# ubc-vision/COTR

Hardware: AMD Instinct MI355X
Metric: query-correspondences/sec at 256x512 SBS, 1k queries (higher is better)
Workload: dtype f32

## Files before the change

cotr_amd/csrc/attention.hip:

```cpp
#include "common.h"

#define ATT_KEYS 512
#define ATT_HD 32

struct AttnFuse {
  const float* x;
  const float* x2;
  const float* wq;
  const float* bq;
  float qscale;
  const float* wo;
  float* part;
  int rows_total;
  int wt;
  unsigned long long* dbg;
};

template <int NS, int QP, bool OP>
__global__ __launch_bounds__(NS * 64) void attention_kernel(const float* __restrict__ q, int ldq,
                                                            const float* __restrict__ k,
                                                            const float* __restrict__ v, int ldkv,
                                                            float* __restrict__ o, int ldo, int nq, int head_major,
                                                            const AttnFuse fz) {
  static_assert(!(QP || OP) || NS == 4 || NS == 8, "the fused variants are written for 4 or 8 key splits");
  constexpr int NBO = 8 / (NS >= 4 ? NS : 4);
  constexpr int SLD = 32 * (NBO > 0 ? NBO : 1) + 4;
  constexpr int QCH = 256 / (NS >= 4 ? NS : 4);
  constexpr int NBLK = ATT_KEYS / NS / 32;
  constexpr int RPW = 16 / NS;
  constexpr int LDS_BUF = OP ? (NS * 32 * SLD > NS * 16 * 64 ? NS * 32 * SLD : NS * 16 * 64) : NS * 16 * 64;
  __shared__ __attribute__((aligned(16))) float lds_buf[LDS_BUF];
  float (*lds_o)[16][64] = reinterpret_cast<float (*)[16][64]>(lds_buf);
  __shared__ float lds_m[NS][32];
  __shared__ float lds_l[NS][32];
  __shared__ __attribute__((aligned(16))) float lds_out[32][36];

  const int t = threadIdx.x;
  const int lane = t & 63, wave = t >> 6;
  const int l31 = lane & 31, hh = lane >> 5;
#define ATT_STAMP(slot)                                                                                                        \
  do {                                                                                                                         \
    if (fz.dbg != nullptr && t == 0) fz.dbg[((size_t)blockIdx.z * gridDim.x + blockIdx.x) * 8 + (slot)] = wall_clock64();      \
  } while (0)
  ATT_STAMP(0);
  const int qtiles = gridDim.x >> 3;
  const int head = head_major ? (blockIdx.x & 7) : (blockIdx.x / qtiles);
  const int qtile = head_major ? (blockIdx.x >> 3) : (blockIdx.x % qtiles);
  const int pair = blockIdx.z;
  const int qi = qtile * 32 + l31;
  const bool q_ok = qi < nq;
  const size_t qrow = (size_t)pair * nq + (q_ok ? qi : 0);

  const size_t key0 = (size_t)pair * ATT_KEYS + (size_t)wave * (ATT_KEYS / NS);
  const float* kg = k + (key0 + l31) * ldkv + head * ATT_HD + hh * 4;
  const float* vg = v + (key0 + 4 * hh) * ldkv + head * ATT_HD + l31;
  f32x4 kf[4];
#pragma unroll
  for (int j = 0; j < 4; ++j) kf[j] = *reinterpret_cast<const f32x4*>(kg + j * 8);
  f32x4 wof[NBO > 0 ? NBO : 1][4];
  if constexpr (OP) {
#pragma unroll
    for (int nb = 0; nb < NBO; ++nb) {
      const float* worow = fz.wo + (size_t)((wave * NBO + nb) * 32 + l31) * 256 + head * ATT_HD + hh * 4;
#pragma unroll
      for (int j = 0; j < 4; ++j) wof[nb][j] = *reinterpret_cast<const f32x4*>(worow + j * 8);
    }
  }

  f32x4 qf[4];
  if constexpr (QP) {
    f32x4 bq4[4];
#pragma unroll
    for (int j = 0; j < 4; ++j) bq4[j] = *reinterpret_cast<const f32x4*>(fz.bq + head * ATT_HD + j * 8 + hh * 4);
    f32x16 qacc;
#pragma unroll
    for (int r = 0; r < 16; ++r) qacc[r] = 0.f;
    constexpr int QJ = QCH / 8;
    const float* wrow = fz.wq + (size_t)(head * ATT_HD + l31) * 256 + wave * QCH + hh * 4;
    const float* xrow = fz.x + qrow * 256 + wave * QCH + hh * 4;
    f32x4 wa[QJ], xb[QJ];
#pragma unroll
    for (int j = 0; j < QJ; ++j) wa[j] = *reinterpret_cast<const f32x4*>(wrow + j * 8);
#pragma unroll
    for (int j = 0; j < QJ; ++j) xb[j] = *reinterpret_cast<const f32x4*>(xrow + j * 8);
    if constexpr (QP == 2) {
      const float* x2row = fz.x2 + qrow * 256 + wave * QCH + hh * 4;
      f32x4 x2b[QJ];
#pragma unroll
      for (int j = 0; j < QJ; ++j) x2b[j] = *reinterpret_cast<const f32x4*>(x2row + j * 8);
#pragma unroll
      for (int j = 0; j < QJ; ++j) xb[j] += x2b[j];
    }
#pragma unroll
    for (int j = 0; j < QJ; ++j)
#pragma unroll
      for (int e = 0; e < 4; ++e) qacc = __builtin_amdgcn_mfma_f32_32x32x2f32(wa[j][e], xb[j][e], qacc, 0, 0, 0);
#pragma unroll
    for (int r = 0; r < 16; ++r) lds_o[wave][r][lane] = qacc[r];
    __syncthreads();
#pragma unroll
    for (int j = 0; j < 4; ++j)
#pragma unroll
      for (int e = 0; e < 4; ++e) {
        const int r = j * 4 + e;
        float sum = 0.f;
#pragma unroll
        for (int w = 0; w < NS; ++w) sum += lds_o[w][r][lane];
        sum += bq4[j][e];
        qf[j][e] = sum * fz.qscale * 1.44269504088896340736f;
      }
    __syncthreads();
    ATT_STAMP(1);
  } else {
#pragma unroll
    for (int j = 0; j < 4; ++j) {
      const f32x4 z = {0.f, 0.f, 0.f, 0.f};
      qf[j] = q_ok ? *reinterpret_cast<const f32x4*>(q + qrow * ldq + head * ATT_HD + j * 8 + hh * 4) : z;
      qf[j] *= 1.44269504088896340736f;
    }
  }
  f32x16 oacc;
#pragma unroll
  for (int r = 0; r < 16; ++r) oacc[r] = 0.f;
  float m_run = -INFINITY, l_run = 0.f;

#pragma unroll
  for (int kb = 0; kb < NBLK; ++kb) {
    float vf[16];
#pragma unroll
    for (int r = 0; r < 16; ++r) vf[r] = vg[(size_t)(kb * 32 + (r & 3) + 8 * (r >> 2)) * ldkv];
    f32x16 s;
#pragma unroll
    for (int r = 0; r < 16; ++r) s[r] = 0.f;
    __builtin_amdgcn_s_setprio(1);
#pragma unroll
    for (int j = 0; j < 4; ++j)
#pragma unroll
      for (int e = 0; e < 4; ++e) s = __builtin_amdgcn_mfma_f32_32x32x2f32(kf[j][e], qf[j][e], s, 0, 0, 0);
    if (kb + 1 < NBLK) {
#pragma unroll
      for (int j = 0; j < 4; ++j) kf[j] = *reinterpret_cast<const f32x4*>(kg + (size_t)(kb + 1) * 32 * ldkv + j * 8);
    }
    __builtin_amdgcn_s_setprio(0);
    float mx = s[0];
#pragma unroll
    for (int r = 1; r < 16; ++r) mx = fmaxf(mx, s[r]);
    mx = fmaxf(mx, __shfl_xor(mx, 32));
    const float m_new = fmaxf(m_run, mx);
    const float alpha = __builtin_amdgcn_exp2f(m_run - m_new);
    float psum = 0.f;
#pragma unroll
    for (int r = 0; r < 16; ++r) {
      s[r] = __builtin_amdgcn_exp2f(s[r] - m_new);
      psum += s[r];
    }
    l_run = l_run * alpha + psum;
    m_run = m_new;
#pragma unroll
    for (int r = 0; r < 16; ++r) oacc[r] *= alpha;
    __builtin_amdgcn_s_setprio(1);
#pragma unroll
    for (int r = 0; r < 16; ++r) oacc = __builtin_amdgcn_mfma_f32_32x32x2f32(vf[r], s[r], oacc, 0, 0, 0);
    __builtin_amdgcn_s_setprio(0);
  }
  l_run += __shfl_xor(l_run, 32);
  ATT_STAMP(2);

#pragma unroll
  for (int r = 0; r < 16; ++r) lds_o[wave][r][lane] = oacc[r];
  if (hh == 0) {
    lds_m[wave][l31] = m_run;
    lds_l[wave][l31] = l_run;
  }
  __syncthreads();
  float m_all = lds_m[0][l31];
#pragma unroll
  for (int w = 1; w < NS; ++w) m_all = fmaxf(m_all, lds_m[w][l31]);
  float f[NS];
  float l_all = 0.f;
#pragma unroll
  for (int w = 0; w < NS; ++w) {
    f[w] = __builtin_amdgcn_exp2f(lds_m[w][l31] - m_all);
    l_all += f[w] * lds_l[w][l31];
  }
  const float inv = 1.f / l_all;
#pragma unroll
  for (int i = 0; i < RPW; ++i) {
    const int r = wave * RPW + i;
    float acc = 0.f;
#pragma unroll
    for (int w = 0; w < NS; ++w) acc += f[w] * lds_o[w][r][lane];
    lds_out[l31][(r & 3) + 8 * (r >> 2) + 4 * hh] = acc * inv;
  }
  __syncthreads();
  ATT_STAMP(3);
  if constexpr (OP) {
    float* stage = lds_buf + wave * (32 * SLD);
    f32x4 af[4];
#pragma unroll
    for (int j = 0; j < 4; ++j) af[j] = *reinterpret_cast<const f32x4*>(&lds_out[l31][j * 8 + hh * 4]);
#pragma unroll
    for (int nb = 0; nb < NBO; ++nb) {
      f32x16 pacc;
#pragma unroll
      for (int r = 0; r < 16; ++r) pacc[r] = 0.f;
#pragma unroll
      for (int j = 0; j < 4; ++j)
#pragma unroll
        for (int e = 0; e < 4; ++e) pacc = __builtin_amdgcn_mfma_f32_32x32x2f32(af[j][e], wof[nb][j][e], pacc, 0, 0, 0);
#pragma unroll
      for (int r = 0; r < 16; ++r) stage[((r & 3) + 8 * (r >> 2) + 4 * hh) * SLD + nb * 32 + l31] = pacc[r];
    }
    ATT_STAMP(4);
    float* pbase = fz.part + ((size_t)head * fz.rows_total + (size_t)pair * nq) * 256 + wave * (32 * NBO);
    constexpr int LPR = 8 * NBO;
    constexpr int RPI = 64 / LPR;
    const int sr = lane / LPR, sc = (lane % LPR) * 4;
#pragma unroll
    for (int it = 0; it < 32 / RPI; ++it) {
      const int row = it * RPI + sr;
      const int qo = qtile * 32 + row;
      const f32x4 val = *reinterpret_cast<const f32x4*>(&stage[row * SLD + sc]);
      if (qo < nq) store_f32x4(pbase + (size_t)qo * 256 + sc, val, fz.wt != 0);
    }
    ATT_STAMP(5);
    if (o == nullptr) return;
  }
  for (int i = t; i < 256; i += NS * 64) {
    const int row = i >> 3, c4 = (i & 7) * 4;
    const int qo = qtile * 32 + row;
    if (qo < nq)
      *reinterpret_cast<f32x4*>(o + ((size_t)pair * nq + qo) * ldo + head * ATT_HD + c4) =
          *reinterpret_cast<const f32x4*>(&lds_out[row][c4]);
  }
}


template <int NS, int OCC>
__global__ __launch_bounds__(NS * 64, OCC) void attention_wide_kernel(const float* __restrict__ q, int ldq,
                                                                 const float* __restrict__ k,
                                                                 const float* __restrict__ v, int ldkv,
                                                                 float* __restrict__ o, int ldo, int nq, int head_major) {
  constexpr int NBLK = ATT_KEYS / NS / 32;
  constexpr int RPW = 16 / NS;
  __shared__ __attribute__((aligned(16))) float lds_o[NS][2][16][64];
  __shared__ float lds_m[NS][2][32];
  __shared__ float lds_l[NS][2][32];
  __shared__ __attribute__((aligned(16))) float lds_out[64][36];
  constexpr bool QL = OCC >= 3;
  __shared__ __attribute__((aligned(16))) f32x4 lds_q[QL ? 2 * 4 * 64 : 1];

  const int t = threadIdx.x;
  const int lane = t & 63, wave = t >> 6;
  const int l31 = lane & 31, hh = lane >> 5;
  const int qtiles = gridDim.x >> 3;
  const int head = head_major ? (blockIdx.x & 7) : (blockIdx.x / qtiles);
  const int qtile = head_major ? (blockIdx.x >> 3) : (blockIdx.x % qtiles);
  const int pair = blockIdx.z;

  const size_t key0 = (size_t)pair * ATT_KEYS + (size_t)wave * (ATT_KEYS / NS);
  const float* kg = k + (key0 + l31) * ldkv + head * ATT_HD + hh * 4;
  const float* vg = v + (key0 + 4 * hh) * ldkv + head * ATT_HD + l31;
  f32x4 kf[4];
#pragma unroll
  for (int j = 0; j < 4; ++j) kf[j] = *reinterpret_cast<const f32x4*>(kg + j * 8);

  f32x4 qf[2][4];
#pragma unroll
  for (int u = 0; u < 2; ++u) {
    const int qi = qtile * 64 + u * 32 + l31;
    const bool q_ok = qi < nq;
    const size_t qrow = (size_t)pair * nq + (q_ok ? qi : 0);
#pragma unroll
    for (int j = 0; j < 4; ++j) {
      qf[u][j] = *reinterpret_cast<const f32x4*>(q + qrow * ldq + head * ATT_HD + j * 8 + hh * 4);
      qf[u][j] *= q_ok ? 1.44269504088896340736f : 0.f;
    }
  }
  if constexpr (QL) {
    if (wave == 0) {
#pragma unroll
      for (int u = 0; u < 2; ++u)
#pragma unroll
        for (int j = 0; j < 4; ++j) lds_q[(u * 4 + j) * 64 + lane] = qf[u][j];
    }
    __syncthreads();
  }
  f32x16 oacc[2];
  float m_run[2], l_run[2];
#pragma unroll
  for (int u = 0; u < 2; ++u) {
#pragma unroll
    for (int r = 0; r < 16; ++r) oacc[u][r] = 0.f;
    m_run[u] = -INFINITY;
    l_run[u] = 0.f;
  }

#pragma unroll 1
  for (int kb = 0; kb < NBLK; ++kb) {
    float vf[16];
#pragma unroll
    for (int r = 0; r < 16; ++r) vf[r] = vg[(size_t)(kb * 32 + (r & 3) + 8 * (r >> 2)) * ldkv];
    f32x16 s[2];
#pragma unroll
    for (int u = 0; u < 2; ++u)
#pragma unroll
      for (int r = 0; r < 16; ++r) s[u][r] = 0.f;
    __builtin_amdgcn_s_setprio(1);
#pragma unroll
    for (int u = 0; u < 2; ++u)
#pragma unroll
      for (int j = 0; j < 4; ++j) {
        const f32x4 qv = QL ? lds_q[(u * 4 + j) * 64 + lane] : qf[u][j];
#pragma unroll
        for (int e = 0; e < 4; ++e) s[u] = __builtin_amdgcn_mfma_f32_32x32x2f32(kf[j][e], qv[e], s[u], 0, 0, 0);
      }
    if (kb + 1 < NBLK) {
#pragma unroll
      for (int j = 0; j < 4; ++j) kf[j] = *reinterpret_cast<const f32x4*>(kg + (size_t)(kb + 1) * 32 * ldkv + j * 8);
    }
    __builtin_amdgcn_s_setprio(0);
#pragma unroll
    for (int u = 0; u < 2; ++u) {
      float mx = s[u][0];
#pragma unroll
      for (int r = 1; r < 16; ++r) mx = fmaxf(mx, s[u][r]);
      mx = fmaxf(mx, __shfl_xor(mx, 32));
      const float m_new = fmaxf(m_run[u], mx);
      const float alpha = __builtin_amdgcn_exp2f(m_run[u] - m_new);
      float psum = 0.f;
#pragma unroll
      for (int r = 0; r < 16; ++r) {
        s[u][r] = __builtin_amdgcn_exp2f(s[u][r] - m_new);
        psum += s[u][r];
      }
      l_run[u] = l_run[u] * alpha + psum;
      m_run[u] = m_new;
#pragma unroll
      for (int r = 0; r < 16; ++r) oacc[u][r] *= alpha;
      __builtin_amdgcn_s_setprio(1);
#pragma unroll
      for (int r = 0; r < 16; ++r) oacc[u] = __builtin_amdgcn_mfma_f32_32x32x2f32(vf[r], s[u][r], oacc[u], 0, 0, 0);
      __builtin_amdgcn_s_setprio(0);
    }
  }

#pragma unroll
  for (int u = 0; u < 2; ++u) {
    l_run[u] += __shfl_xor(l_run[u], 32);
#pragma unroll
    for (int r = 0; r < 16; ++r) lds_o[wave][u][r][lane] = oacc[u][r];
    if (hh == 0) {
      lds_m[wave][u][l31] = m_run[u];
      lds_l[wave][u][l31] = l_run[u];
    }
  }
  __syncthreads();
#pragma unroll
  for (int u = 0; u < 2; ++u) {
    float m_all = lds_m[0][u][l31];
#pragma unroll
    for (int w = 1; w < NS; ++w) m_all = fmaxf(m_all, lds_m[w][u][l31]);
    float f[NS];
    float l_all = 0.f;
#pragma unroll
    for (int w = 0; w < NS; ++w) {
      f[w] = __builtin_amdgcn_exp2f(lds_m[w][u][l31] - m_all);
      l_all += f[w] * lds_l[w][u][l31];
    }
    const float inv = 1.f / l_all;
#pragma unroll
    for (int i = 0; i < RPW; ++i) {
      const int r = wave * RPW + i;
      float acc = 0.f;
#pragma unroll
      for (int w = 0; w < NS; ++w) acc += f[w] * lds_o[w][u][r][lane];
      lds_out[u * 32 + l31][(r & 3) + 8 * (r >> 2) + 4 * hh] = acc * inv;
    }
  }
  __syncthreads();
  for (int i = t; i < 512; i += NS * 64) {
    const int row = i >> 3, c4 = (i & 7) * 4;
    const int qo = qtile * 64 + row;
    if (qo < nq)
      *reinterpret_cast<f32x4*>(o + ((size_t)pair * nq + qo) * ldo + head * ATT_HD + c4) =
          *reinterpret_cast<const f32x4*>(&lds_out[row][c4]);
  }
}

constexpr size_t ATT_RES_SMEM = (size_t)2 * ATT_KEYS * ATT_HD * sizeof(float);
__global__ __launch_bounds__(512) void attention_res_kernel(const float* __restrict__ q, int ldq, const float* __restrict__ k,
                                                            const float* __restrict__ v, int ldkv, float* __restrict__ o, int ldo, int nq,
                                                            int tiles_per_chunk) {
  extern __shared__ __attribute__((aligned(16))) float res_smem[];
  float* k_s = res_smem;
  float* v_s = res_smem + ATT_KEYS * ATT_HD;
  const int t = threadIdx.x, lane = t & 63, wave = t >> 6;
  const int l31 = lane & 31, hh = lane >> 5;
  const int head = blockIdx.x & 7, chunk = blockIdx.x >> 3;
  const int pair = blockIdx.z;
  {
    const size_t krow0 = (size_t)pair * ATT_KEYS;
    const int c4 = t & 7;
#pragma unroll 4
    for (int r0 = 0; r0 < ATT_KEYS; r0 += 64) {
      const int row = r0 + (t >> 3);
      const f32x4 kk = *reinterpret_cast<const f32x4*>(k + (krow0 + row) * ldkv + head * ATT_HD + c4 * 4);
      const f32x4 vv = *reinterpret_cast<const f32x4*>(v + (krow0 + row) * ldkv + head * ATT_HD + c4 * 4);
      *reinterpret_cast<f32x4*>(k_s + row * ATT_HD + ((c4 ^ (row & 7)) << 2)) = kk;
      *reinterpret_cast<f32x4*>(v_s + row * ATT_HD + ((c4 ^ (row & 7)) << 2)) = vv;
    }
  }
  __syncthreads();
  const int ntiles = (nq + 31) / 32;
  const int t_end = (chunk + 1) * tiles_per_chunk < ntiles ? (chunk + 1) * tiles_per_chunk : ntiles;
  for (int qt = chunk * tiles_per_chunk + wave; qt < t_end; qt += 8) {
    const int qi = qt * 32 + l31;
    const bool q_ok = qi < nq;
    const size_t qrow = (size_t)pair * nq + (q_ok ? qi : 0);
    f32x4 qf[4];
#pragma unroll
    for (int j = 0; j < 4; ++j) {
      qf[j] = *reinterpret_cast<const f32x4*>(q + qrow * ldq + head * ATT_HD + j * 8 + hh * 4);
      qf[j] *= q_ok ? 1.44269504088896340736f : 0.f;
    }
    f32x16 oacc[4];
    float m_run[4], l_run[4];
#pragma unroll
    for (int c = 0; c < 4; ++c) {
#pragma unroll
      for (int r = 0; r < 16; ++r) oacc[c][r] = 0.f;
      m_run[c] = -INFINITY;
      l_run[c] = 0.f;
    }
#pragma unroll 1
    for (int kb = 0; kb < 4; ++kb) {
#pragma unroll
      for (int c = 0; c < 4; ++c) {
        const int key0 = c * 128 + kb * 32;
        const int krow = key0 + l31;
        f32x16 s;
#pragma unroll
        for (int r = 0; r < 16; ++r) s[r] = 0.f;
#pragma unroll
        for (int j = 0; j < 4; ++j) {
          const f32x4 kf = *reinterpret_cast<const f32x4*>(k_s + krow * ATT_HD + (((j * 2 + hh) ^ (krow & 7)) << 2));
#pragma unroll
          for (int e = 0; e < 4; ++e) s = __builtin_amdgcn_mfma_f32_32x32x2f32(kf[e], qf[j][e], s, 0, 0, 0);
        }
        float mx = s[0];
#pragma unroll
        for (int r = 1; r < 16; ++r) mx = fmaxf(mx, s[r]);
        mx = fmaxf(mx, __shfl_xor(mx, 32));
        const float m_new = fmaxf(m_run[c], mx);
        const float alpha = __builtin_amdgcn_exp2f(m_run[c] - m_new);
        float psum = 0.f;
#pragma unroll
        for (int r = 0; r < 16; ++r) {
          s[r] = __builtin_amdgcn_exp2f(s[r] - m_new);
          psum += s[r];
        }
        l_run[c] = l_run[c] * alpha + psum;
        m_run[c] = m_new;
#pragma unroll
        for (int r = 0; r < 16; ++r) oacc[c][r] *= alpha;
#pragma unroll
        for (int r = 0; r < 16; ++r) {
          const int vr = key0 + (r & 3) + 8 * (r >> 2) + 4 * hh;
          const float vf = v_s[vr * ATT_HD + ((((l31 >> 2) ^ (vr & 7)) << 2) | (l31 & 3))];
          oacc[c] = __builtin_amdgcn_mfma_f32_32x32x2f32(vf, s[r], oacc[c], 0, 0, 0);
        }
      }
    }
#pragma unroll
    for (int c = 0; c < 4; ++c) l_run[c] += __shfl_xor(l_run[c], 32);
    float m_all = m_run[0];
#pragma unroll
    for (int c = 1; c < 4; ++c) m_all = fmaxf(m_all, m_run[c]);
    float f[4];
    float l_all = 0.f;
#pragma unroll
    for (int c = 0; c < 4; ++c) {
      f[c] = __builtin_amdgcn_exp2f(m_run[c] - m_all);
      l_all += f[c] * l_run[c];
    }
    const float inv = 1.f / l_all;
    if (q_ok) {
      float* dst = o + qrow * ldo + head * ATT_HD + 4 * hh;
#pragma unroll
      for (int g = 0; g < 4; ++g) {
        f32x4 out;
#pragma unroll
        for (int i = 0; i < 4; ++i) {
          float acc = 0.f;
#pragma unroll
          for (int c = 0; c < 4; ++c) acc += f[c] * oacc[c][g * 4 + i];
          out[i] = acc * inv;
        }
        *reinterpret_cast<f32x4*>(dst + 8 * g) = out;
      }
    }
  }
}

static const int g_att_wide_head_major = 1;

static thread_local unsigned long long* g_att_dbg = nullptr;
void set_attention_debug_times(unsigned long long* p) { g_att_dbg = p; }
static thread_local const char* g_att_variant = "";
const char* attention_last_variant() { return g_att_variant; }
static const int g_att_part_wt = 1;

int init_attention_attributes() { return 0; }

int launch_attention(const float* q, int ldq, const float* k, const float* v, int ldkv, float* o, int ldo,
                     int nb, int nq, hipStream_t s) {
  if (nb <= 0 || nq <= 0) return 0;
  if (ldq % 4 || ldkv % 4 || ldo % 4) return -1;
  int ns = knob(KN_ATTENTION_SPLITS);
  const int g_att_head_major = (knob(KN_XCD_MAPPING) >> 3) & 1;
  const long g_att_wide_min_rows = knob(KN_ATTENTION_WIDE_MIN_ROWS);
  const int g_att_resident = knob(KN_ATTENTION_RESIDENT), g_att_wide_occ = knob(KN_ATTENTION_WIDE_OCCUPANCY) == 2 ? 2 : 3;
  const int res_tiles = (nq + 31) / 32;
  int res_tpc = 32;
  while (res_tpc > 8 && (long)((res_tiles + res_tpc - 1) / res_tpc) * 8 * nb < 256) res_tpc /= 2;
  const long res_wgs = (long)((res_tiles + res_tpc - 1) / res_tpc) * 8 * nb;
  if (ns == 0 && g_att_resident && (long)nb * nq >= g_att_wide_min_rows && nq >= 256 && res_wgs >= 128) {
    static PerDeviceFlag attr_set;
    if (!attr_set.get()) {
      if (hipFuncSetAttribute(reinterpret_cast<const void*>(attention_res_kernel), hipFuncAttributeMaxDynamicSharedMemorySize,
                              (int)ATT_RES_SMEM) != hipSuccess)
        return -2;
      attr_set.set();
    }
    const int chunks = (res_tiles + res_tpc - 1) / res_tpc;
    g_att_variant = "res";
    hipLaunchKernelGGL(attention_res_kernel, dim3(chunks * 8, 1, nb), dim3(512), ATT_RES_SMEM, s, q, ldq, k, v, ldkv, o, ldo, nq, res_tpc);
    return hipGetLastError() == hipSuccess ? 0 : -2;
  }
  if (ns == 0 && (long)nb * nq >= g_att_wide_min_rows) {
    dim3 wgrid(((nq + 63) / 64) * 8, 1, nb);
    g_att_variant = g_att_wide_occ == 3 ? "wide3" : "wide2";
    if (g_att_wide_occ == 3)
      hipLaunchKernelGGL((attention_wide_kernel<4, 3>), wgrid, dim3(256), 0, s, q, ldq, k, v, ldkv, o, ldo, nq, g_att_wide_head_major);
    else
      hipLaunchKernelGGL((attention_wide_kernel<4, 2>), wgrid, dim3(256), 0, s, q, ldq, k, v, ldkv, o, ldo, nq, g_att_wide_head_major);
    return hipGetLastError() == hipSuccess ? 0 : -2;
  }
  dim3 grid(((nq + 31) / 32) * 8, 1, nb);
  AttnFuse fz = {};
  if (ns == 0) ns = 4;
  switch (ns) {
    case 1:
      g_att_variant = "s1";
      hipLaunchKernelGGL((attention_kernel<1, 0, false>), grid, dim3(64), 0, s, q, ldq, k, v, ldkv, o, ldo, nq, g_att_head_major, fz);
      break;
    case 2:
      g_att_variant = "s2";
      hipLaunchKernelGGL((attention_kernel<2, 0, false>), grid, dim3(128), 0, s, q, ldq, k, v, ldkv, o, ldo, nq, g_att_head_major, fz);
      break;
    case 4:
      g_att_variant = "s4";
      hipLaunchKernelGGL((attention_kernel<4, 0, false>), grid, dim3(256), 0, s, q, ldq, k, v, ldkv, o, ldo, nq, g_att_head_major, fz);
      break;
    case 8:
      g_att_variant = "s8";
      hipLaunchKernelGGL((attention_kernel<8, 0, false>), grid, dim3(512), 0, s, q, ldq, k, v, ldkv, o, ldo, nq, g_att_head_major, fz);
      break;
    case 16:
      g_att_variant = "s16";
      hipLaunchKernelGGL((attention_kernel<16, 0, false>), grid, dim3(1024), 0, s, q, ldq, k, v, ldkv, o, ldo, nq, g_att_head_major, fz);
      break;
    default:
      return -1;
  }
  return hipGetLastError() == hipSuccess ? 0 : -2;
}

#define ATT_CT_PARAM
static int attention_fused_impl(const float* q, int ldq, const float* x, const float* x2, const float* wq, const float* bq,
                                float qscale, const float* k, const float* v, int ldkv, float* o, int ldo, const float* wo,
                                float* part, int nb, int nq, hipStream_t s ATT_CT_PARAM) {
  if (nb <= 0 || nq <= 0) return 0;
  const bool qp = wq != nullptr, op = wo != nullptr;
  const int g_att_head_major = (knob(KN_XCD_MAPPING) >> 3) & 1;
  const int g_att_fused_splits = knob(KN_ATTENTION_FUSED_SPLITS);
  if (ldkv % 4 || (o && ldo % 4) || (!qp && (q == nullptr || ldq % 4))) return -1;
  if (qp && (bq == nullptr || (x == nullptr && x2 == nullptr))) return -1;
  if (op && part == nullptr) return -1;
  if (!op && o == nullptr) return -1;
  dim3 grid(((nq + 31) / 32) * 8, 1, nb);
  AttnFuse fz = {};
  fz.x = x ? x : x2; fz.x2 = x ? x2 : nullptr; fz.wq = wq; fz.bq = bq; fz.qscale = qscale;
  fz.wo = wo; fz.part = part; fz.rows_total = nb * nq; fz.wt = g_att_part_wt;
  fz.dbg = g_att_dbg;
  const int qmode = !qp ? 0 : (fz.x2 ? 2 : 1);
  const int ns = g_att_fused_splits == 48 ? (qp ? 8 : 4) : g_att_fused_splits == 84 ? (qp ? 4 : 8) : g_att_fused_splits ? g_att_fused_splits : 4;
#define ATT_LAUNCH(NSV, QPV, OPV)                                                                                         \
  hipLaunchKernelGGL((attention_kernel<NSV, QPV, OPV>), grid, dim3(NSV * 64), 0, s, q, ldq, k, v, ldkv, o, ldo, nq, g_att_head_major, fz)
#define ATT_PICK(NSV)                              \
  do {                                             \
    if (qmode == 2 && op) ATT_LAUNCH(NSV, 2, true);   \
    else if (qmode == 2) ATT_LAUNCH(NSV, 2, false);   \
    else if (qmode == 1 && op) ATT_LAUNCH(NSV, 1, true); \
    else if (qmode == 1) ATT_LAUNCH(NSV, 1, false);   \
    else if (op) ATT_LAUNCH(NSV, 0, true);            \
    else ATT_LAUNCH(NSV, 0, false);                   \
  } while (0)
  g_att_variant = ns == 8 ? "s8" : "s4";
  if (ns == 8) ATT_PICK(8);
  else ATT_PICK(4);
#undef ATT_PICK
#undef ATT_LAUNCH
  return hipGetLastError() == hipSuccess ? 0 : -2;
}

int launch_attention_fused(const float* q, int ldq, const float* x, const float* x2, const float* wq, const float* bq,
                           float qscale, const float* k, const float* v, int ldkv, float* o, int ldo, const float* wo,
                           float* part, int nb, int nq, hipStream_t s) {
  return attention_fused_impl(q, ldq, x, x2, wq, bq, qscale, k, v, ldkv, o, ldo, wo, part, nb, nq, s);
}
```

Measured before the change: 1.214 million.

## Add 16-query-tile attention kernel for small grids that underfill CUs

Adds an attention kernel that handles 16 queries per block instead of 32 across 4 key splits, with K, V and the optional output-projection weights preloaded into registers and MFMA 16x16x4 f32 used for QK, PV and the output projection. It is dispatched only when Q is not fused, the split count is 4, and the original grid has fewer blocks than there are CUs, so that doubling the block count can fill more of the device. The trade-off is more redundant K/V loads per query and high register pressure from the preloaded operands.

Measured after the change: 1.241 million, median of 6. 1.02x the previous value.

```diff
diff --git a/cotr_amd/csrc/attention.hip b/cotr_amd/csrc/attention.hip
--- a/cotr_amd/csrc/attention.hip
+++ b/cotr_amd/csrc/attention.hip
@@ -229,6 +229,185 @@
   for (int i = t; i < 256; i += NS * 64) {
     const int row = i >> 3, c4 = (i & 7) * 4;
     const int qo = qtile * 32 + row;
+    if (qo < nq)
+      *reinterpret_cast<f32x4*>(o + ((size_t)pair * nq + qo) * ldo + head * ATT_HD + c4) =
+          *reinterpret_cast<const f32x4*>(&lds_out[row][c4]);
+  }
+}
+
+
+template <bool OP>
+__global__ __launch_bounds__(256) void attention_q16_kernel(const float* __restrict__ q, int ldq, const float* __restrict__ k,
+                                                            const float* __restrict__ v, int ldkv, float* __restrict__ o, int ldo,
+                                                            int nq, int head_major, const AttnFuse fz) {
+  constexpr int NS = 4, KPW = ATT_KEYS / NS, NBLK = KPW / 64;
+  constexpr int SLD = 64 + 4;
+  constexpr int LDS_BUF = (OP && NS * 16 * SLD > NS * 8 * 64) ? NS * 16 * SLD : NS * 8 * 64;
+  __shared__ __attribute__((aligned(16))) float lds_buf[LDS_BUF];
+  float (*lds_o)[8][64] = reinterpret_cast<float (*)[8][64]>(lds_buf);
+  __shared__ float lds_m[NS][16];
+  __shared__ float lds_l[NS][16];
+  __shared__ __attribute__((aligned(16))) float lds_out[16][36];
+
+  const int t = threadIdx.x;
+  const int lane = t & 63, wave = t >> 6;
+  const int l15 = lane & 15, g = lane >> 4;
+  const int qtiles = gridDim.x >> 3;
+  const int head = head_major ? (blockIdx.x & 7) : (blockIdx.x / qtiles);
+  const int qtile = head_major ? (blockIdx.x >> 3) : (blockIdx.x % qtiles);
+  const int pair = blockIdx.z;
+  const int qi = qtile * 16 + l15;
+  const bool q_ok = qi < nq;
+  const size_t qrow = (size_t)pair * nq + (q_ok ? qi : 0);
+  const size_t key0 = (size_t)pair * ATT_KEYS + (size_t)wave * KPW;
+
+  f32x4 qf[2];
+#pragma unroll
+  for (int j = 0; j < 2; ++j) qf[j] = *reinterpret_cast<const f32x4*>(q + qrow * ldq + head * ATT_HD + g * 8 + j * 4);
+  f32x4 kf[NBLK][4][2];
+  float vf[NBLK][2][16];
+#pragma unroll
+  for (int kb = 0; kb < NBLK; ++kb) {
+#pragma unroll
+    for (int tt = 0; tt < 4; ++tt) {
+      const float* kg = k + (key0 + kb * 64 + tt * 16 + l15) * ldkv + head * ATT_HD + g * 8;
+      kf[kb][tt][0] = *reinterpret_cast<const f32x4*>(kg);
+      kf[kb][tt][1] = *reinterpret_cast<const f32x4*>(kg + 4);
+    }
+#pragma unroll
+    for (int r = 0; r < 16; ++r) {
+      const float* vg = v + (key0 + kb * 64 + (r >> 2) * 16 + 4 * g + (r & 3)) * ldkv + head * ATT_HD + l15;
+      vf[kb][0][r] = vg[0];
+      vf[kb][1][r] = vg[16];
+    }
+  }
+  f32x4 wof[4][2];
+  if constexpr (OP) {
+#pragma unroll
+    for (int nt = 0; nt < 4; ++nt) {
+      const float* worow = fz.wo + (size_t)(wave * 64 + nt * 16 + l15) * 256 + head * ATT_HD + g * 8;
+      wof[nt][0] = *reinterpret_cast<const f32x4*>(worow);
+      wof[nt][1] = *reinterpret_cast<const f32x4*>(worow + 4);
+    }
+  }
+  __builtin_amdgcn_sched_barrier(0);
+#pragma unroll
+  for (int j = 0; j < 2; ++j) {
+    const f32x4 z = {0.f, 0.f, 0.f, 0.f};
+    qf[j] = q_ok ? qf[j] * 1.44269504088896340736f : z;
+  }
+
+  f32x4 oacc[2];
+#pragma unroll
+  for (int dh = 0; dh < 2; ++dh)
+#pragma unroll
+    for (int i = 0; i < 4; ++i) oacc[dh][i] = 0.f;
+  float m_run = -INFINITY, l_run = 0.f;
+#pragma unroll
+  for (int kb = 0; kb < NBLK; ++kb) {
+    f32x4 s[4];
+#pragma unroll
+    for (int tt = 0; tt < 4; ++tt)
+#pragma unroll
+      for (int i = 0; i < 4; ++i) s[tt][i] = 0.f;
+#pragma unroll
+    for (int j = 0; j < 2; ++j)
+#pragma unroll
+      for (int e = 0; e < 4; ++e)
+#pragma unroll
+        for (int tt = 0; tt < 4; ++tt) s[tt] = __builtin_amdgcn_mfma_f32_16x16x4f32(kf[kb][tt][j][e], qf[j][e], s[tt], 0, 0, 0);
+    float mx = s[0][0];
+#pragma unroll
+    for (int tt = 0; tt < 4; ++tt)
+#pragma unroll
+      for (int i = 0; i < 4; ++i) mx = fmaxf(mx, s[tt][i]);
+    mx = fmaxf(mx, __shfl_xor(mx, 16));
+    mx = fmaxf(mx, __shfl_xor(mx, 32));
+    const float m_new = fmaxf(m_run, mx);
+    const float alpha = __builtin_amdgcn_exp2f(m_run - m_new);
+    float psum = 0.f;
+#pragma unroll
+    for (int tt = 0; tt < 4; ++tt)
+#pragma unroll
+      for (int i = 0; i < 4; ++i) {
+        s[tt][i] = __builtin_amdgcn_exp2f(s[tt][i] - m_new);
+        psum += s[tt][i];
+      }
+    l_run = l_run * alpha + psum;
+    m_run = m_new;
+#pragma unroll
+    for (int dh = 0; dh < 2; ++dh) oacc[dh] *= alpha;
+#pragma unroll
+    for (int r = 0; r < 16; ++r)
+#pragma unroll
+      for (int dh = 0; dh < 2; ++dh) oacc[dh] = __builtin_amdgcn_mfma_f32_16x16x4f32(vf[kb][dh][r], s[r >> 2][r & 3], oacc[dh], 0, 0, 0);
+  }
+  l_run += __shfl_xor(l_run, 16);
+  l_run += __shfl_xor(l_run, 32);
+
+#pragma unroll
+  for (int dh = 0; dh < 2; ++dh)
+#pragma unroll
+    for (int i = 0; i < 4; ++i) lds_o[wave][dh * 4 + i][lane] = oacc[dh][i];
+  if (g == 0) {
+    lds_m[wave][l15] = m_run;
+    lds_l[wave][l15] = l_run;
+  }
+  __syncthreads();
+  float m_all = lds_m[0][l15];
+#pragma unroll
+  for (int w = 1; w < NS; ++w) m_all = fmaxf(m_all, lds_m[w][l15]);
+  float f[NS];
+  float l_all = 0.f;
+#pragma unroll
+  for (int w = 0; w < NS; ++w) {
+    f[w] = __builtin_amdgcn_exp2f(lds_m[w][l15] - m_all);
+    l_all += f[w] * lds_l[w][l15];
+  }
+  const float inv = 1.f / l_all;
+#pragma unroll
+  for (int i = 0; i < 2; ++i) {
+    const int r = wave * 2 + i;
+    float acc = 0.f;
+#pragma unroll
+    for (int w = 0; w < NS; ++w) acc += f[w] * lds_o[w][r][lane];
+    lds_out[l15][(r >> 2) * 16 + 4 * g + (r & 3)] = acc * inv;
+  }
+  __syncthreads();
+  if constexpr (OP) {
+    float* stage = lds_buf + wave * (16 * SLD);
+    f32x4 af[2];
+#pragma unroll
+    for (int j = 0; j < 2; ++j) af[j] = *reinterpret_cast<const f32x4*>(&lds_out[l15][g * 8 + j * 4]);
+    f32x4 pacc[4];
+#pragma unroll
+    for (int nt = 0; nt < 4; ++nt)
+#pragma unroll
+      for (int i = 0; i < 4; ++i) pacc[nt][i] = 0.f;
+#pragma unroll
+    for (int j = 0; j < 2; ++j)
+#pragma unroll
+      for (int e = 0; e < 4; ++e)
+#pragma unroll
+        for (int nt = 0; nt < 4; ++nt) pacc[nt] = __builtin_amdgcn_mfma_f32_16x16x4f32(af[j][e], wof[nt][j][e], pacc[nt], 0, 0, 0);
+#pragma unroll
+    for (int nt = 0; nt < 4; ++nt)
+#pragma unroll
+      for (int i = 0; i < 4; ++i) stage[(4 * g + i) * SLD + nt * 16 + l15] = pacc[nt][i];
+    float* pbase = fz.part + ((size_t)head * fz.rows_total + (size_t)pair * nq) * 256 + wave * 64;
+    const int sr = lane >> 4, sc = (lane & 15) * 4;
+#pragma unroll
+    for (int it = 0; it < 4; ++it) {
+      const int row = it * 4 + sr;
+      const int qo = qtile * 16 + row;
+      const f32x4 val = *reinterpret_cast<const f32x4*>(&stage[row * SLD + sc]);
+      if (qo < nq) store_f32x4(pbase + (size_t)qo * 256 + sc, val, fz.wt != 0);
+    }
+    if (o == nullptr) return;
+  }
+  if (t < 128) {
+    const int row = t >> 3, c4 = (t & 7) * 4;
+    const int qo = qtile * 16 + row;
     if (qo < nq)
       *reinterpret_cast<f32x4*>(o + ((size_t)pair * nq + qo) * ldo + head * ATT_HD + c4) =
           *reinterpret_cast<const f32x4*>(&lds_out[row][c4]);
@@ -596,6 +775,15 @@
   fz.dbg = g_att_dbg;
   const int qmode = !qp ? 0 : (fz.x2 ? 2 : 1);
   const int ns = g_att_fused_splits == 48 ? (qp ? 8 : 4) : g_att_fused_splits == 84 ? (qp ? 4 : 8) : g_att_fused_splits ? g_att_fused_splits : 4;
+  if (!qp && ns == 4 && (long)grid.x * nb < cotr_num_cus()) {
+    dim3 grid16(((nq + 15) / 16) * 8, 1, nb);
+    g_att_variant = "q16";
+    if (op)
+      hipLaunchKernelGGL((attention_q16_kernel<true>), grid16, dim3(256), 0, s, q, ldq, k, v, ldkv, o, ldo, nq, g_att_head_major, fz);
+    else
+      hipLaunchKernelGGL((attention_q16_kernel<false>), grid16, dim3(256), 0, s, q, ldq, k, v, ldkv, o, ldo, nq, g_att_head_major, fz);
+    return hipGetLastError() == hipSuccess ? 0 : -2;
+  }
 #define ATT_LAUNCH(NSV, QPV, OPV)                                                                                         \
   hipLaunchKernelGGL((attention_kernel<NSV, QPV, OPV>), grid, dim3(NSV * 64), 0, s, q, ldq, k, v, ldkv, o, ldo, nq, g_att_head_major, fz)
 #define ATT_PICK(NSV)                              \
```
